# tomer196/GaUDI

Hardware: AMD Instinct MI355X
Metric: guided molecules/sec (1000-step) (higher is better)
Workload: dtype f32

## Files before the change

gaudi_amd/csrc/w8_nodes_f16.h:

```cpp
#pragma once
#include "w8_split.h"

namespace gaudi {
namespace w8 {


constexpr float kLoScale = 2048.f;
#ifndef GAUDI_NODE_ABLATE
#define GAUDI_NODE_ABLATE 0
#endif
constexpr int kAblateH = GAUDI_NODE_ABLATE;
#ifndef GAUDI_NODE_STAMPS
#define GAUDI_NODE_STAMPS 0
#endif
#ifndef GAUDI_NODE_PRIO
#define GAUDI_NODE_PRIO 1
#endif
struct NodeStampH {
  unsigned long long sum[8], last;
  __device__ __forceinline__ void start() { last = __builtin_amdgcn_s_memtime(); }
  __device__ __forceinline__ void mark(int i) {
    const unsigned long long t = __builtin_amdgcn_s_memtime();
    sum[i] += t - last;
    last = t;
// ... 140 lines not shown
  NodeSetH<NodeGeoH<HP>::NTW> s[NodeGeoH<HP>::D];
};

constexpr int kOOBBytes = (int)0x80000000u;
template <int HP>
struct TileLanesH {
  int vo[NodeGeoH<HP>::NTW];
  __device__ __forceinline__ TileLanesH(int wave, int lane, bool on = true) {
#pragma unroll
    for (int u = 0; u < NodeGeoH<HP>::NTW; ++u)
      vo[u] = (on && wave + kWaves * u < NodeGeoH<HP>::T) ? lane * 16 + (wave + kWaves * u) * 2048 : kOOBBytes;
  }
};
template <int HP, int NU = NodeGeoH<HP>::NTW>
__device__ __forceinline__ void nh_load(NodeSetH<NodeGeoH<HP>::NTW>& s, const WBuf& wh, int chunk_off, const TileLanesH<HP>& tl) {
#pragma unroll
  for (int u = 0; u < NU; ++u) {
    s.p[u][0] = __builtin_bit_cast(u4, __builtin_amdgcn_raw_buffer_load_b128(wh.r, tl.vo[u], chunk_off * 4, GAUDI_NODE_LOAD_AUX));
    s.p[u][1] = __builtin_bit_cast(u4, __builtin_amdgcn_raw_buffer_load_b128(wh.r, tl.vo[u] + 1024, chunk_off * 4, GAUDI_NODE_LOAD_AUX));
  }
}
constexpr int kAheadOne = 1, kAheadAll = 99;
template <int HP, int AHEAD = kAheadAll, int NU = 0>
__device__ __forceinline__ void node_prefetch_h(NodePFH<HP>& pf, const WBuf& wh, int W , int wave, int lane) {
  constexpr int nd = AHEAD < NodeGeoH<HP>::D ? AHEAD : NodeGeoH<HP>::D;
  const TileLanesH<HP> tl(wave, lane);
  static_for<nd>([&](auto d_tag) {
    constexpr int d = decltype(d_tag)::value;
    nh_load<HP, (NU > 0 ? NU : NodeGeoH<HP>::NTW)>(pf.s[d], wh, 2 * W + d * nh_chunk_floats(HP), tl);
  });
}

constexpr int kNodePlain = 0;
constexpr int kNodeFresh = 1;
constexpr int kNodeOneTile = 2;
constexpr int kNodeSlots1 = 4, kNodeSlots2 = 8;
__host__ __device__ constexpr bool node_one_tile(int FL) { return (FL & 3) == kNodeOneTile; }
template <int HP>
__host__ __device__ constexpr bool node_uneven_slots() { return NodeGeoH<HP>::NTW == 2 && NodeGeoH<HP>::T < 2 * kWaves; }
template <int HP>
__host__ __device__ constexpr int node_slots(int FL) { return node_one_tile(FL) && node_uneven_slots<HP>() ? FL >> 2 : 0; }
constexpr int kTailRuntime = 0;
constexpr int kTailOne = 1;

struct NodeCtxH {
  float winv;
  float* split_a;
  float* split_b;
  bool ktail;
  float* scales;
  float* scales_b = nullptr;
};

struct YInitBias {};
struct YInitRows {
  const float* y;
};
template <int HP, int EPI, bool TWO, int MAXNT, int PIN = kAheadOne, int POUT = kAheadOne, int FL = kNodePlain, int TAIL = kTailRuntime,
          int NU = 0, class XB = const float*, class XA = const float*, class YI = YInitBias>
__device__ __forceinline__ void node_gemm_h(const WBuf& wh, int Wa, const XA& sXa, bool do_split_a, int Wb, const XB& sXb,
                                            const float* sBias, float* sY, const float* sRes, const float* sMask, int N, int wave,
                                            int lane, const NodeCtxH& cx, NodePFH<HP>& pf, int nextW = -1, float* gPre = nullptr,
                                            uint32_t* sMaxOut = nullptr ,
                                            NodeStampH* ns = nullptr, const YI& yinit = YI{}) {
  (void)ns;
  (void)yinit;
  using G = NodeGeoH<HP>;
  constexpr int T = G::T, LD = HP + 4, NTW = NU > 0 ? NU : G::NTW, nc = G::nc, D = G::D;
  constexpr int kIn = PIN < D ? PIN : D, kOut = POUT < D ? POUT : D;
  constexpr int TQ = TAIL == kTailOne ? 1 : 4;
  const bool ktail = TAIL == kTailOne ? true : cx.ktail;
  constexpr bool kFresh = FL == kNodeFresh;
  const int c = lane & 15, g = lane >> 4;
  const int nt = (MAXNT < 2 || N <= 16) ? 1 : (MAXNT < 3 || N <= 32) ? 2 : 3;
  const bool seq = TWO && cx.split_b == cx.split_a;
  const SplitBufH sa{cx.split_a, nt, cx.scales}, sb{cx.split_b, nt, cx.scales_b != nullptr ? cx.scales_b : cx.scales + kScaleFloatsH};
  const int bpos = nh_bpos(c, g);
  const TileLanesH<HP> tl(wave, lane);
  const TileLanesH<HP> tl_next(wave, lane, nextW >= 0);
  const int Wn = nextW >= 0 ? nextW : Wa;
  static_for<D>([&](auto d_tag) {
    constexpr int d = decltype(d_tag)::value;
    if constexpr (d >= kIn) nh_load<HP, NTW>(pf.s[d], wh, 2 * Wa + d * nh_chunk_floats(HP), tl);
  });
  float ta[NTW][TQ], tb[NTW][TQ];
  if constexpr (G::odd) {
#pragma unroll
    for (int u = 0; u < NTW; ++u) {
      const int t = wave + kWaves * u < T ? wave + kWaves * u : 0;
#pragma unroll
      for (int q = 0; q < TQ; ++q) {
        const int ln = ((q == 0 || !ktail) && wave + kWaves * u < T) ? lane : kOOBLane;
        ta[u][q] = __builtin_bit_cast(float, __builtin_amdgcn_raw_buffer_load_b32(wh.r, ln * 4, (2 * Wa + nh_tail_off(HP) + t * 256 + q * 64) * 4, 0));
        if constexpr (TWO)
          tb[u][q] = __builtin_bit_cast(float, __builtin_amdgcn_raw_buffer_load_b32(wh.r, ln * 4, (2 * Wb + nh_tail_off(HP) + t * 256 + q * 64) * 4, 0));
      }
    }
  }
  NSTAMP(0);
  if (!(kAblateH & 1)) {
    const int ls = kFresh ? fresh(lane) : lane;
    if (do_split_a) split_rows_h<HP>(sa, rows_of(sXa), N, wave, ls);
    if (TWO && !seq) split_rows_h<HP>(sb, sXb, N, wave, ls);
    NSTAMP(1);
    if (do_split_a || (TWO && !seq)) lds_barrier();
    NSTAMP(2);
  }

  f4 acc0[MAXNT][NTW], acc1[MAXNT][NTW], y[MAXNT][NTW];
#pragma unroll
  for (int j = 0; j < MAXNT; ++j)
#pragma unroll
    for (int u = 0; u < NTW; ++u) {
      const int t = wave + kWaves * u < T ? wave + kWaves * u : 0;
      acc0[j][u] = splat(0.f);
      acc1[j][u] = splat(0.f);
      y[j][u] = sBias != nullptr ? *(const f4*)(sBias + 16 * t + 4 * g) : splat(0.f);
      if constexpr (std::is_same<YI, YInitRows>::value)
        y[j][u] = j * 16 + c < N ? *(const f4*)(yinit.y + (j * 16 + c) * LD + 16 * t + 4 * g) : splat(0.f);
// ... 3 lines not shown
  };
  auto bld = [&](const SplitBufH& s_, int i, int j) {
    const float* q = s_.chunk(i) + bpos + j * 512;
    return BH{*(const u4*)q, *(const u4*)(q + 256)};
  };
  auto mm = [&](const NodeSetH<G::NTW>& s, const BH& b, int j) {
    if (kAblateH & 2) {
      asm volatile("" ::"v"(s.p[0][0]), "v"(s.p[0][1]), "v"(s.p[NTW - 1][0]), "v"(s.p[NTW - 1][1]), "v"(b.h), "v"(b.l));
      return;
    }
#pragma unroll
    for (int u = 0; u < NTW; ++u) acc1[j][u] = mfma_h(s.p[u][0], b.l, acc1[j][u]);
#pragma unroll
    for (int u = 0; u < NTW; ++u) acc0[j][u] = mfma_h(s.p[u][0], b.h, acc0[j][u]);
#pragma unroll
    for (int u = 0; u < NTW; ++u) acc1[j][u] = mfma_h(s.p[u][1], b.h, acc1[j][u]);
  };
  auto tail_steps = [&](const SplitBufH& s_, const float (&tw)[NTW][TQ], auto j_tag) {
    constexpr int j = decltype(j_tag)::value;
    if constexpr (G::odd) {
      const float* xt = s_.tail(HP) + j * 256 + g * 16 + c;
#pragma unroll
      for (int u = 0; u < NTW; ++u) y[j][u] = mfma1(tw[u][0], xt[0], y[j][u]);
      if constexpr (TQ > 1) {
        if (!ktail) {
#pragma unroll
          for (int q = 1; q < TQ; ++q)
#pragma unroll
            for (int u = 0; u < NTW; ++u) y[j][u] = mfma1(tw[u][q], xt[64 * q], y[j][u]);
        }
      }
    }
  };
  auto fold = [&](const SplitBufH& s_, const float (&tw)[NTW][TQ]) {
    static_for<MAXNT>([&](auto j_tag) {
      constexpr int j = decltype(j_tag)::value;
      if (j < nt) {
        tail_steps(s_, tw, j_tag);
        const float sc = s_.scale(HP)[j * 16 + c] * cx.winv;
#pragma unroll
        for (int u = 0; u < NTW; ++u) {
          y[j][u] = y[j][u] + (acc0[j][u] + acc1[j][u] * (1.0f / kLoScale)) * sc;
          acc0[j][u] = splat(0.f);
          acc1[j][u] = splat(0.f);
        }
      }
    });
  };
  auto source = [&](auto src_tag, const SplitBufH& s_) {
    constexpr int src = decltype(src_tag)::value;
    constexpr bool last_src = !TWO || src == 1;
    const int Wcur = src == 0 ? Wa : Wb;
    BH bcur = bld(s_, 0, 0);
    static_for<nc>([&](auto i_tag) {
      constexpr int i = decltype(i_tag)::value;
      constexpr int d = i % D;
      BH bnext = bcur;
      if constexpr (i + 1 < nc) bnext = bld(s_, i + 1, 0);
      __builtin_amdgcn_sched_barrier(0);
      mm(pf.s[d], bcur, 0);
      if constexpr (MAXNT >= 2) {
        if (nt >= 2) {
          mm(pf.s[d], bld(s_, i, 1), 1);
          if constexpr (MAXNT >= 3) {
            if (nt >= 3) mm(pf.s[d], bld(s_, i, 2), 2);
          }
        }
      }
      __builtin_amdgcn_sched_barrier(0);
      if (!(kAblateH & 4)) {
        if constexpr (i + D < nc) nh_load<HP, NTW>(pf.s[d], wh, 2 * Wcur + (i + D) * nh_chunk_floats(HP), tl);
        else if constexpr (!last_src) nh_load<HP, NTW>(pf.s[d], wh, 2 * Wb + d * nh_chunk_floats(HP), tl);
        else if constexpr (d < kOut) nh_load<HP, NTW>(pf.s[d], wh, 2 * Wn + d * nh_chunk_floats(HP), tl_next);
      }
      __builtin_amdgcn_sched_barrier(0);
      bcur = bnext;
    });
  };
  NSTAMP(3);
#if GAUDI_NODE_PRIO
  if constexpr (!kFresh)
    if ((GAUDI_NODE_PRIO == 1 && wave >= kWaves / 2) || (GAUDI_NODE_PRIO == 2 && wave < kWaves / 2)) __builtin_amdgcn_s_setprio(1);
#endif
  source(std::integral_constant<int, 0>{}, sa);
  NSTAMP(4);
  fold(sa, ta);
  NSTAMP(5);
  if constexpr (TWO) {
    if (seq) {
      lds_barrier();
      split_rows_h<HP>(sb, sXb, N, wave, kFresh ? fresh(lane) : lane);
      lds_barrier();
    }
    source(std::integral_constant<int, 1>{}, sb);
    fold(sb, tb);
  }
#if GAUDI_NODE_PRIO
  if constexpr (!kFresh) __builtin_amdgcn_s_setprio(0);
#endif
  const int le = kFresh ? fresh(lane) : lane, ce = le & 15, ge = le >> 4;
  static_for<MAXNT>([&](auto j_tag) {
    constexpr int j = decltype(j_tag)::value;
    if (j < nt) {
#pragma unroll
      for (int u = 0; u < NTW; ++u) {
        const int t = wave + kWaves * u;
        const int nd = j * 16 + ce;
        f4 yy = y[j][u];
        if (t < T && nd < N) {
          float* dst = sY + nd * LD + 16 * t + 4 * ge;
          const bool pad = G::odd && ktail && t == T - 1 && ge > 0;
          if (pad) yy = splat(0.f);
          if (gPre != nullptr) nstash_store((f4*)(gPre + nd * HP + 16 * t + 4 * ge), yy);
          if (sMaxOut != nullptr) atomicMax(sMaxOut + nd, umax(umax(absbits(yy[0]), absbits(yy[1])), umax(absbits(yy[2]), absbits(yy[3]))));
          if (!pad) {
            if (EPI == EPI_SILU) yy = silu4v(yy);
            if (EPI == EPI_RESIDUAL_MASK) {
              const f4 r = *(const f4*)(sRes + nd * LD + 16 * t + 4 * ge);
              yy = (r + yy) * sMask[nd];
            }
            if (EPI == EPI_MUL_DSILU) {
              const f4 r = *(const f4*)(sRes + nd * LD + 16 * t + 4 * ge);
              yy = yy * dsilu4v(r);
            }
            if (EPI == EPI_ACCUM) yy = *(const f4*)(sRes + nd * LD + 16 * t + 4 * ge) + yy;
          }
          *(f4*)dst = yy;
        }
// ... 74 lines not shown
        f4 y = a.bias != nullptr ? *(const f4*)(a.bias + 16 * t + 4 * g) : splat(0.f);
        if constexpr (G::odd) y = mfma1(job.tw[u], xt, y);
        y = y + (job.acc0[u] + job.acc1[u] * (1.0f / kLoScale)) * sc;
        if (c < a.N) *(f4*)(a.out + c * LD + 16 * t + 4 * g) = y;
      });
    }
  }
}
template <int HP, int S>
__device__ __forceinline__ void side_rest(SideJobH<HP>& job, const SideArgsH& a, int lane) {
  if constexpr (S < SideGeoH<HP>::kSteps) {
    side_compute<HP, S>(job, a, lane);
    __builtin_amdgcn_sched_barrier(0);
    side_issue<HP, S + 1>(job, a, lane);
    side_rest<HP, S + 1>(job, a, lane);
  }
}
template <int HP, int MODE, int S0>
__device__ __forceinline__ void side_trips(RingS<HP, MODE>& ring, const WBuf& wb, int W, int nextW, int lane, SideJobH<HP>& job,
                                           const SideArgsH& a) {
  static_for<side_trip_count<HP, MODE>()>([&](auto tr_tag) {
    constexpr int tr = decltype(tr_tag)::value, s = S0 + tr;
    side_barrier<SideGeoH<HP>::loads(s)>();
    RingsStageSide<HP, MODE, tr>::run(ring, wb, W, nextW, lane);
    __builtin_amdgcn_sched_barrier(0);
    side_compute<HP, s>(job, a, lane);
    __builtin_amdgcn_sched_barrier(0);
    side_issue<HP, s + 1>(job, a, lane);
    __builtin_amdgcn_sched_barrier(0);
    ring.par ^= 1;
  });
}

#ifndef GAUDI_NODE_F16
#define GAUDI_NODE_F16 1
#endif
template <int SP>
struct NodeMath {
  static constexpr bool kF16 = SP != 0 && GAUDI_NODE_F16 != 0;
};
template <int HP, bool NH>
struct NodePFSel {
  using type = NodePF<HP>;
};
template <int HP>
struct NodePFSel<HP, true> {
  using type = NodePFH<HP>;
};
template <int HP, bool NH, int AHEAD, int FL = kNodePlain, class PF>
__device__ __forceinline__ void node_prefetch_x(PF& pf, const WBuf& wb, const WBuf& wbe, int W, int N, int wave, int lane, bool tw) {
  if constexpr (NH) node_prefetch_h<HP, AHEAD, node_slots<HP>(FL)>(pf, wbe, W, wave, lane);
  else node_prefetch<HP>(pf, wb, W, wave, lane, tw);
}
template <int HP, int EPI, bool TWO, int GN, bool NH, int PIN, int POUT, int FL = kNodePlain, int XBS = 0, class PF>
__device__ __forceinline__ void node_gemm_x(const WBuf& wb, const WBuf& wbe, int Wa, const float* Xa, const float* XaS, bool split_a, int Wb,
                                            const float* Xb, const float* XbS, const float* sBias, float* sY, const float* sRes,
                                            const float* sMask, int N, int wave, int lane, bool tw, const NodeCtxH& cx, PF& pf,
                                            int nextW = -1, float* gPre = nullptr, uint32_t* sMaxOut = nullptr,
                                            const float* Xb1 = nullptr, float xb_div = 1.f) {
  static_assert(XBS == 0 || (NH && GN == 0 && TWO), "summed second sources: the fp16-pair form of the resident kernels");
  if constexpr (NH) {
    constexpr int MAXNT = GN ? 3 : node_one_tile(FL) ? 1 : 2;
    constexpr int TAIL = node_one_tile(FL) && nh_odd(HP) ? kTailOne : kTailRuntime;
    constexpr int NU = node_slots<HP>(FL);
    if constexpr (XBS == 0)
      node_gemm_h<HP, EPI, TWO, MAXNT, PIN, POUT, FL, TAIL, NU>(wbe, Wa, Xa, split_a, Wb, Xb, sBias, sY, sRes, sMask, N, wave, lane, cx, pf, nextW,
                                                                gPre, sMaxOut);
    else
      node_gemm_h<HP, EPI, TWO, MAXNT, PIN, POUT, FL, TAIL, NU>(wbe, Wa, Xa, split_a, Wb, RowsSum<XBS == 2>{Xb, Xb1, xb_div}, sBias, sY, sRes, sMask,
                                                                N, wave, lane, cx, pf, nextW, gPre, sMaxOut);
  } else if constexpr (GN != 0) {
    node_gemm_n<HP, EPI, true, 3>(wb, Wa, XaS, Wb, XbS, sBias, sY, sRes, sMask, N, wave, lane, tw, &pf, nextW, gPre);
  } else {
    node_gemm<HP, EPI, true>(wb, Wa, Xa, Wb, Xb, sBias, sY, sRes, sMask, N, wave, lane, tw, &pf, nextW, gPre);
  }
}
__host__ __device__ constexpr bool node_ring_idle(int HP, int SP, bool GN) {
  return GN || (SP != 0 && GAUDI_NODE_F16 != 0 && (SP == 2 || HP < 48));
}
template <int HP>
__device__ __forceinline__ NodeCtxH node_ctx_h(float* region, int cap, int N, float winv, bool ktail, float* scales) {
  const int nct = N <= 16 ? 1 : N <= 32 ? 2 : 3;
  const int need = nh_split_floats(HP, nct);
  return NodeCtxH{winv, region, 2 * need <= cap ? region + need : region, ktail, scales};
}
__host__ __device__ constexpr int nh_keep_floats(int HP, int N) { return nh_split_floats(HP, N <= 16 ? 1 : N <= 32 ? 2 : 3) + kScaleFloatsH; }
template <int HP>
__device__ __forceinline__ NodeCtxH node_ctx_keep(const NodeCtxH& cx, float* keep, int N) {
  const int nct = N <= 16 ? 1 : N <= 32 ? 2 : 3;
  return NodeCtxH{cx.winv, keep + kScaleFloatsH, cx.split_a, cx.ktail, keep, cx.scales};
  (void)nct;
}

}
}
```

gaudi_amd/csrc/w8_pred.h:

```cpp
#pragma once
#include "pred_device.h"
#include "w8_edm.h"

namespace gaudi {
namespace w8 {

template <int HP, int SP = 0, int GN = 0, bool PG = false>
struct PredSmem {
  static_assert(!(PG && GN != 0), "PG is a variant of the resident kernels");
  static_assert(!GN || SP != 0, "global node buffers: split edge GEMMs only (the fp32 form's publish buffer starts in b0 / b1)");
  static constexpr bool kGlobalNodes = GN != 0;
  float *b2, *b3, *b4;
  float *b0, *b1;
  float* ring;
  float* pub;
  float *x, *x0, *dx;
  uint32_t *pmax, *qmax;
  float* hsc;
  f4* geo;
  float *d0, *trans, *dd0;
  float* pred;
  float* vec;
  float* hk = nullptr;
  float* side = nullptr;
  __host__ __device__ static int floats(int N, int S, int pubx) {
    return EdgeRing<HP, SP>::kFloats + (GN ? gn_lds_buffers(GN) : PG ? 4 : 5) * N * (HP + 4) + pubx + 12 * N + 2 * align4(N) + 96 + S * 10 + 32 + 10 * HP;
  }
  __device__ __forceinline__ float* publish() const { return GN ? ring : b0; }
  __device__ void carve(float* base, int N, int S, int pubx, float* gnode = nullptr) {
    constexpr int LD = HP + 4;
    if (SP == 0) { ring = base; base += EdgeRing<HP, SP>::kFloats; }
    if (GN || PG) gnode = assume_global(gnode);
    float*& nb = GN ? gnode : base;
    if (GN == 2) { b2 = base; base += N * LD; } else { b2 = nb; nb += N * LD; }
    b3 = nb; nb += N * LD;
    if (PG) { b4 = gnode; gnode += N * LD; } else { b4 = nb; nb += N * LD; }
    b0 = nb; nb += N * LD;
    if (GN == 2) { b1 = base; base += N * LD; } else { b1 = nb; nb += N * LD; }
    if (SP != 0) { ring = base; base += EdgeRing<HP, SP>::kFloats; }
    pub = base; base += pubx;
    x = base; base += 4 * N;
    x0 = base; base += 4 * N;
    dx = base; base += 4 * N;
    pmax = (uint32_t*)base; base += align4(N);
    qmax = (uint32_t*)base; base += align4(N);
    hsc = base; base += 96;
    geo = (f4*)base; base += S * 4;
    d0 = base; base += S;
    trans = base; base += S * 4;
    dd0 = base; base += S;
    pred = base; base += 32;
    vec = base;
  }
};

// ... 212 lines not shown
    STAMP(ST_BARRIER);
    vec_prefetch<NV, kThreads>(vpf, wb, PredLayerW::vec_off(lay.layer(l + 1 < W.L ? l + 1 : l), HP), PredLayerW::vec_count(HP), tid);
    if constexpr (STG) {
      stage_rows(xs0, p, N * LD, wave, lane);
      stage_wait();
    }
    node_gemm_x<HP, EPI_RESIDUAL_MASK, false, GN, NH, kAheadOne, kAheadOne, FL>(wb, wbe, Lw.Wn2, p, xs0, true, -1, nullptr, nullptr, Lw.bn2, h, h, mg.mask, mg.NC, wave,
                                                     lane, tw, hctx(), pf, l + 1 < W.L ? lay.layer(l + 1) : -1);
    if (!last) coord_update(sm, mg, 1.0f, tid);
    STAMP(ST_NODE);
    __syncthreads();
    STAMP(ST_BARRIER);
  }
  {
    const float* ow = w + lay.out_w();
    const float* ob = w + lay.out_b();
    const float* msk = mg.mask;
    small_dots<kThreads>(
        N * K, HP, tid, [=](int qq, int f) { return gload(ow + (qq % K) * HP + f); },
        [=](int qq, int f) { return h[(qq / K) * LD + f]; },
        [=](int qq, float acc) { p[qq] = (acc + gload(ob + qq % K)) * msk[qq / K]; });
    __syncthreads();
    if (tid < K) {
      float s = 0.f;
      for (int n = 0; n < N; ++n) s += p[n * K + tid];
      sm.pred[tid] = s / readout_div;
    }
    __syncthreads();
  }
  STAMP(ST_X0);
}

template <int HP, int SP = 0, bool MR = false, int GN = 0, int FL = 0, class SM = PredSmem<HP, SP, GN>>
__device__ __forceinline__ void pred_backward(const PredDev& W, const MolGraph& mg, const SM& sm, const float* stash,
                                              float* sGrad, float readout_div, int pub_ch, int tid STAMP_DECL, const float* sZin = nullptr) {
  constexpr int LD = HP + 4;
  constexpr int T = HP / 16;
  const int wave = __builtin_amdgcn_readfirstlane(tid >> 6), lane = tid & 63, c = lane & 15, g = lane >> 4;
  const int N = mg.N, D = mg.D, F = W.F, F1 = F + 1, K = W.K, S = mg.S;
  PredLayout lay{HP, F1, K, W.L};
  const float* __restrict__ w = W.w;
  const WBuf wb = make_wbuf(W.w, W.w_bytes);
  const WBuf wbe = SP ? make_wbuf(W.ws, W.ws_bytes) : wb;
  const bool tw = W.ktail != 0;
  float *B0 = sm.b0, *B1 = sm.b1, *B2 = sm.b2, *dh = sm.b3, *B4 = sm.b4;
  const int tid_ = tid;
  float* pub = sm.publish();
  const int PLD = 16 * pub_ch + 4;
  const float* estash = stash + pred_stash_node_floats(N, HP, W.L);
  const float* astash = estash + (size_t)W.L * S * HP * 2;
  const float* pstash = astash + (size_t)W.L * S;
  const float* dpred = sm.pred + 16;
  const int nslots = mg.ntiles * 16;
  f4* dus = (f4*)const_cast<float*>(pstash + (size_t)W.L * S);

  if (sZin != nullptr) {
    for (int idx = tid; idx < N * 3; idx += kThreads) {
      const int n = idx / 3, d = idx % 3;
      const float v = sZin[n * D + d] * mg.mask[n];
      sm.x[4 * n + d] = v;
      sm.x0[4 * n + d] = v;
    }
    __syncthreads();
    compute_geo(sm, mg, 0.f, tid, true);
    __syncthreads();
  }
  {
    const float* ow = w + lay.out_w();
    for (int idx = tid; idx < N * HP; idx += kThreads) {
      const int n = idx / HP, f = idx % HP;
      float acc = 0.f;
      for (int k = 0; k < K; ++k) acc += (dpred[k] / readout_div) * gload(ow + k * HP + f);
      dh[n * LD + f] = acc * mg.mask[n];
    }
    for (int idx = tid; idx < N * 4; idx += kThreads) sm.dx[idx] = 0.f;
    for (int idx = tid; idx < S; idx += kThreads) sm.dd0[idx] = 0.f;
  }
  __syncthreads();

  typename EdgeRing<HP, SP>::type ring;
  er_init<HP>(ring, sm.ring, W.ktail != 0, W.ws, W.hinv);
  constexpr bool NH = NodeMath<SP>::kF16;
  constexpr bool RI = node_ring_idle(HP, SP, GN);
  constexpr bool STG = GN && !NH;
  float* const xs0 = sm.ring;
  float* const xs1 = sm.ring + stage_stride(N * LD);
  if constexpr (!RI) {
    const int L0 = lay.layer(W.L - 1);
    er_start<HP>(ring, wbe, L0 + 9 * HP * HP , wave, lane);
  }
  typename NodePFSel<HP, NH>::type pf;
  node_prefetch_x<HP, NH, kAheadOne, FL>(pf, wb, wbe, lay.layer(W.L - 1) + 13 * HP * HP , mg.NC, wave, lane, tw);
  auto hctx = [&]() {
    if constexpr (NH) {
      if constexpr (RI) return node_ctx_h<HP>(sm.ring, EdgeRing<HP, SP>::kFloats, mg.NC, W.hinv, tw, sm.hsc);
      else return node_ctx_h<HP>(ring.slot(ring.par ^ 1), EdgeRing<HP, SP>::kFloats / 2, mg.NC, W.hinv, tw, sm.hsc);
    } else {
      return NodeCtxH{1.f, nullptr, nullptr, tw, nullptr};
    }
  };
  constexpr int NV = (PredLayerW::vec_count(HP) + kThreads - 1) / kThreads;
  VecPF<NV> vpf;
  vec_prefetch<NV, kThreads>(vpf, wb, PredLayerW::vec_off(lay.layer(W.L - 1), HP), PredLayerW::vec_count(HP), tid);
  STAMP(ST_X1);
  for (int l = W.L - 1; l >= 0; --l) {
    const bool last = l == W.L - 1;
    const PredLayerW Lw(w, lay.layer(l), HP, sm.vec);
    const float* st = stash + (size_t)l * (3 * N * HP + 4 * N);
    {
      const int tid = fresh(tid_);
      const int n4 = N * (HP / 4);
#ifdef GAUDI_DIAG_HOT_STASH
      const f4* sp = (const f4*)W.w;
      const f4* sq = (const f4*)(W.w + N * HP);
      const f4* sn = (const f4*)(W.w + 2 * N * HP);
#else
      const f4* sp = (const f4*)st;
      const f4* sq = (const f4*)(st + N * HP);
      const f4* sn = (const f4*)(st + 2 * N * HP);
#endif
      const int i0 = tid < n4 ? tid : n4 - 1, i1 = tid + kThreads < n4 ? tid + kThreads : n4 - 1;
      const f4 xv = gload4((const f4*)(st + 3 * N * HP) + (tid < N ? tid : N - 1));
      const f4 p0 = nstash_load(sp + i0), q0 = nstash_load(sq + i0), v0 = nstash_load(sn + i0);
      const f4 p1 = nstash_load(sp + i1), q1 = nstash_load(sq + i1), v1 = nstash_load(sn + i1);
      vec_commit<NV, kThreads>(vpf, sm.vec, PredLayerW::vec_count(HP), tid);
      STAMP(ST_GUIDE);
      auto put = [&](int idx, f4 pv, f4 qv, f4 nv) {
        const int n = idx / (HP / 4), f = 4 * (idx % (HP / 4));
        *(f4*)(B2 + n * LD + f) = pv;
        *(f4*)(B1 + n * LD + f) = qv;
        *(f4*)(B4 + n * LD + f) = nv;
        *(f4*)(dh + n * LD + f) = *(const f4*)(dh + n * LD + f) * mg.mask[n];
      };
      if (tid < N) {
        *(f4*)(sm.x + 4 * tid) = xv;
        *(f4*)(sm.dx + 4 * tid) = *(const f4*)(sm.dx + 4 * tid) * mg.mask[tid];
      }
      if (tid < n4) put(tid, p0, q0, v0);
      if (tid + kThreads < n4) put(tid + kThreads, p1, q1, v1);
      for (int idx = tid + 2 * kThreads; idx < n4; idx += kThreads) put(idx, nstash_load(sp + idx), nstash_load(sq + idx), nstash_load(sn + idx));
      for (int idx = tid + kThreads; idx < N; idx += kThreads) {
        *(f4*)(sm.x + 4 * idx) = gload4((const f4*)(st + 3 * N * HP) + idx);
        *(f4*)(sm.dx + 4 * idx) = *(const f4*)(sm.dx + 4 * idx) * mg.mask[idx];
      }
    }
    STAMP(ST_PRED_IO);
    __syncthreads();
    if constexpr (STG) stage_rows(xs0, dh, N * LD, wave, lane);
    compute_geo(sm, mg, 1.0f, tid, false);
    if constexpr (STG) stage_wait();
    STAMP(ST_BWD_EDGE);
    node_gemm_x<HP, EPI_MUL_DSILU, false, GN, NH, kAheadOne, kAheadOne, FL>(wb, wbe, Lw.Wn2t, dh, xs0, true, -1, nullptr, nullptr, nullptr, STG ? xs1 : B4, B4, nullptr,
                                                 mg.NC, wave, lane, tw, hctx(), pf, Lw.Wn1ht);
    __syncthreads();
    {
      const NodeCtxH cx = hctx();
      node_gemm_x<HP, EPI_ACCUM, false, GN, NH, kAheadOne, kAheadAll, FL>(wb, wbe, Lw.Wn1ht, B4, xs1, true, -1, nullptr, nullptr, nullptr, dh, dh, nullptr, mg.NC,
                                                     wave, lane, tw, cx, pf, Lw.Wn1at);
      node_gemm_x<HP, EPI_NONE, false, GN, NH, kAheadAll, 0, FL>(wb, wbe, Lw.Wn1at, B4, xs1, false, -1, nullptr, nullptr, nullptr, B0, nullptr, nullptr,
                                                    mg.NC, wave, lane, tw, cx, pf);
    }
    __syncthreads();
    STAMP(ST_BWD_NODE);
    if constexpr (RI) er_start<HP>(ring, wbe, last ? Lw.W2t : Lw.Wc1t, wave, lane);
    {
      constexpr bool mr = MR;
      int rd = 0;
    pred_bwd_round:
      const bool more = MR && rd + 1 < mg.rounds;
      const TileCols tc = load_tile(mg, MR ? rd : 0, wave, c);
      const int tile = tc.slot >> 4;
      const f4 gg = sm.geo[tc.slot];
      const float d0v = sm.d0[tc.slot];
      f4 du[T];
      float a = 0.f, tau = 0.f, dtx = 0.f, dty = 0.f, dtz = 0.f;
      {
        f4 de[T];
        if (tc.active) {
          a = gload(astash + (size_t)l * S + tc.slot);
          dtx = sm.dx[4 * tc.i + 0];
          dty = sm.dx[4 * tc.i + 1];
          dtz = sm.dx[4 * tc.i + 2];
        }
        if (!last) {
          f4 cp[T];
          if (tc.active) {
#ifdef GAUDI_DIAG_HOT_STASH
            const f4* sc = (const f4*)(W.w + (size_t)tile * (T * 256)) + lane;
#else
            const f4* sc = (const f4*)(estash + edge_stash_off8(l, tile, 1, S, HP)) + lane;
#endif
#pragma unroll
            for (int t = 0; t < T; ++t) cp[t] = stash_load(sc + t * 64);
            const float phi = gload(pstash + (size_t)l * S + tc.slot);
            const float th = tanhf(phi);
            tau = W.use_tanh ? th * W.coords_range_layer : phi;
            const float dtau = (dtx * gg[1] + dty * gg[2] + dtz * gg[3]) * tc.mk;
            const float dphi = W.use_tanh ? dtau * W.coords_range_layer * (1.0f - th * th) : dtau;
#pragma unroll
            for (int t = 0; t < T; ++t)
              cp[t] = *(const f4*)(Lw.wc2 + 16 * t + 4 * g) * dphi * cp[t];
          } else {
#pragma unroll
            for (int t = 0; t < T; ++t) cp[t] = splat(0.f);
          }
          STAMP(ST_B_DCP);
          er_gemm_regs<HP>(de, cp, ring, wbe, Lw.Wc1t, Lw.W2t, nullptr, B0 + tc.i * LD ,
                             tc.active, wave, lane);
          STAMP(ST_B_DE);
        } else {
#pragma unroll
          for (int t = 0; t < T; ++t) de[t] = *(const f4*)(B0 + tc.i * LD + 16 * t + 4 * g);
        }
        if (tc.active) {
          f4 ve[T];
#ifdef GAUDI_DIAG_HOT_STASH
          const f4* sv = (const f4*)(W.w + (size_t)(8 + tile) * (T * 256)) + lane;
#else
          const f4* sv = (const f4*)(estash + edge_stash_off8(l, tile, 0, S, HP)) + lane;
#endif
#pragma unroll
          for (int t = 0; t < T; ++t) ve[t] = stash_load(sv + t * 64);
          float dadot = 0.f;
#pragma unroll
          for (int t = 0; t < T; ++t) dadot += dot4(de[t], silu4v(ve[t]));
          const float da = reduce_groups(dadot) * tc.mk;
          const float ds = W.attention ? da * a * (1.0f - a) : 0.f;
          const float am = a * tc.mk;
#pragma unroll
          for (int t = 0; t < T; ++t)
            de[t] = (de[t] * am + *(const f4*)(Lw.wa + 16 * t + 4 * g) * ds) * dsilu4v(ve[t]);
        }
        STAMP(ST_B_DV);
        er_gemm_regs<HP>(du, de, ring, wbe, Lw.W2t,
                         more ? (last ? Lw.W2t : Lw.Wc1t) : ((SP == 0 && l > 0) ? lay.layer(l - 1) + 10 * HP * HP : -1), nullptr, nullptr,
                         tc.active, wave, lane);
        STAMP(ST_B_DT1);
      }
      if (tc.active) {
        const float* pp = B2 + tc.i * LD + 4 * g;
        const float* qq = B1 + tc.j * LD + 4 * g;
        float drdot = 0.f, dd0dot = 0.f;
#pragma unroll
        for (int t = 0; t < T; ++t) {
          const f4 u = edge_u(pp, qq, Lw.cr, Lw.cd, g, t, gg[0], d0v);
          du[t] = du[t] * dsilu4v(u);
          drdot += dot4(du[t], *(const f4*)(Lw.cr + 16 * t + 4 * g));
          dd0dot += dot4(du[t], *(const f4*)(Lw.cd + 16 * t + 4 * g));
        }
        const float dr = reduce_groups(drdot), dd0v = reduce_groups(dd0dot);
        if (g == 0) {
          const int i = tc.i, j = tc.j;
          const float fx = sm.x[4 * i + 0] - sm.x[4 * j + 0];
          const float fy = sm.x[4 * i + 1] - sm.x[4 * j + 1];
          const float fz = sm.x[4 * i + 2] - sm.x[4 * j + 2];
          const float nrm = sqrtf(gg[0] + 1e-8f), den = nrm + 1.0f;
          const float cx = dtx * tau * tc.mk, cy = dty * tau * tc.mk, cz = dtz * tau * tc.mk;
          const float k1 = (cx * fx + cy * fy + cz * fz) / (den * den * nrm);
          *(f4*)(sm.trans + 4 * tc.slot) = (f4){cx / den - fx * k1 + 2.0f * fx * dr, cy / den - fy * k1 + 2.0f * fy * dr,
                                                cz / den - fz * k1 + 2.0f * fz * dr, 0.f};
          sm.dd0[tc.slot] += dd0v;
        }
      }
      if constexpr (MR) {
        if (more) {
          if (tc.active) {
            f4* sd = dus + (size_t)tile * (T * 64) + lane;
#pragma unroll
            for (int t = 0; t < T; ++t) stash_store(sd + t * 64, du[t]);
          }
          ++rd;
          goto pred_bwd_round;
        }
      }
      STAMP(ST_B_DU);
// ... 192 lines not shown
```

gaudi_amd/csrc/w8_split.h:

```cpp
#pragma once
#include "w8_common.h"
#ifndef GAUDI_EDGE_PRIO
#define GAUDI_EDGE_PRIO 0
#endif


namespace gaudi {
namespace w8 {

typedef _Float16 h8 __attribute__((ext_vector_type(8)));
typedef _Float16 h2 __attribute__((ext_vector_type(2)));
typedef __attribute__((ext_vector_type(2))) float f2;
typedef __attribute__((ext_vector_type(4))) uint32_t u4;
typedef __attribute__((ext_vector_type(2))) uint32_t u2;
constexpr int kPieces = 2;

template <int N, class F>
__device__ __forceinline__ void static_for(F f) {
  if constexpr (N > 0) {
    static_for<N - 1>(f);
    f(std::integral_constant<int, N - 1>{});
  }
}

// ... 250 lines not shown
  auto gen = [&](int m) {
    const f4 lo = silu4v(edge_u(pp, qq, sCr, sCd, g, 2 * m, r, d0));
    const f4 hi = 2 * m + 1 < T ? silu4v(edge_u(pp, qq, sCr, sCd, g, 2 * m + 1 < T ? 2 * m + 1 : 0, r, d0)) : splat(0.f);
    return split8(lo, hi, se);
  };
  B3 bin = gen(0), nb = bin;
  static_assert(G::NH <= 3, "at most three trips per K chunk");
  const bool tail = G::kTailOK && ring.ktail;
#if GAUDI_EDGE_PRIO & 1
  if (wave >= kWaves / 2) __builtin_amdgcn_s_setprio(1);
#endif
  auto chunk = [&](int m, const B3& bin, B3& nb) {
    const int mn = m + 1 < G::NC ? m + 1 : m;
    auto trip = [&](auto h_tag) {
      constexpr int h = decltype(h_tag)::value;
      constexpr int NT = G::tiles_of(h);
      const int tr = m * G::NH + h;
      trip_open(ring, lane);
      rings_mfma<HP, MODE, NT>(acc + h * G::CH, ring.slot(ring.par) + lane * 4, bin, active, [&] {
        rings_stage(ring, wb, W, nextW, tr, wave, lane);
        if (h == G::NH - 1) nb = gen(mn);
      });
      trip_close(ring, lane);
    };
    trip(std::integral_constant<int, 0>{});
    if constexpr (G::NH > 1) trip(std::integral_constant<int, 1>{});
    if constexpr (G::NH > 2) trip(std::integral_constant<int, 2>{});
  };
  const int full = tail ? G::NC - 1 : G::NC;
  int m = 0;
#pragma unroll 1
  for (; m + 1 < full; m += 2) {
    chunk(m, bin, nb);
    chunk(m + 1, nb, bin);
  }
  if (m < full) chunk(m, bin, nb);
  if constexpr (G::kTailOK) {
    if (tail) {
      trip_open(ring, lane);
      const float bt = silu_f(edge_u_tail(pp, qq, sCr, sCd, g, T, r, d0)[0]) * se;
      rings_mfma_tail<HP, MODE>(acc, ring.slot(ring.par) + lane * 4, bt, active,
                          [&] { rings_stage(ring, wb, W, nextW, G::kTripsTail - 1, wave, lane); });
      trip_close(ring, lane);
    }
  }
#if GAUDI_EDGE_PRIO & 1
  __builtin_amdgcn_s_setprio(0);
#endif
  const float dsc = sc.inv * ring.winv;
#pragma unroll
  for (int t = 0; t < T; ++t) acc[t] = acc[t] * dsc + *(const f4*)(sB2 + 16 * t + 4 * g);
}

template <int HP, int MODE>
__device__ __forceinline__ void edge_gemm_regs_s(f4 (&out)[HP / 16], const f4 (&in)[HP / 16], RingS<HP, MODE>& ring, const WBuf& wb,
                                                 int W, int nextW, const float* sBias, const float* rowinit, bool active,
                                                 int wave, int lane) {
  using G = SplitGeo<HP, MODE>;
  constexpr int T = G::T;
  const int g = lane >> 4;
  uint32_t mx = 0;
#pragma unroll
  for (int t = 0; t < T; ++t) {
    out[t] = splat(0.f);
    mx = umax(mx, umax(umax(absbits(in[t][0]), absbits(in[t][1])), umax(absbits(in[t][2]), absbits(in[t][3]))));
  }
  const Pow2Scale sc = scale_for(column_max(mx));
  const float se = sc.s;
  static_assert(G::NH <= 3, "at most three trips per K chunk");
  const int c = lane & 15;
#if GAUDI_EDGE_PRIO & 2
  if (wave >= kWaves / 2) __builtin_amdgcn_s_setprio(1);
#endif
  auto chunk = [&](auto m_tag) {
    constexpr int m = decltype(m_tag)::value;
    const B3 bin = split8(in[2 * m], 2 * m + 1 < T ? in[2 * m + 1 < T ? 2 * m + 1 : 0] : splat(0.f), se);
    auto trip = [&](auto h_tag) {
      constexpr int h = decltype(h_tag)::value;
      constexpr int tr = m * G::NH + h;
      trip_open(ring, lane);
      rings_mfma<HP, MODE, G::tiles_of(h)>(out + h * G::CH, ring.slot(ring.par) + lane * 4, bin, active,
                                           [&] { rings_stage(ring, wb, W, nextW, tr, wave, lane); });
      trip_close(ring, lane);
    };
    trip(std::integral_constant<int, 0>{});
    if constexpr (G::NH > 1) trip(std::integral_constant<int, 1>{});
    if constexpr (G::NH > 2) trip(std::integral_constant<int, 2>{});
  };
  auto finish = [&] {
#if GAUDI_EDGE_PRIO & 2
    __builtin_amdgcn_s_setprio(0);
#endif
    const float dsc = sc.inv * ring.winv;
#pragma unroll
    for (int t = 0; t < T; ++t) {
      f4 b = sBias != nullptr ? *(const f4*)(sBias + 16 * t + 4 * g) : splat(0.f);
      if (rowinit != nullptr) b = b + *(const f4*)(rowinit + 16 * t + 4 * g);
      out[t] = out[t] * dsc + b;
    }
  };
  static_for<G::NC - 1>([&](auto m_tag) { chunk(m_tag); });
  if constexpr (G::kTailOK) {
    if (ring.ktail) {
      trip_open(ring, lane);
      rings_mfma_tail<HP, MODE>(out, ring.slot(ring.par) + lane * 4, tail_to_b(in[T - 1], c, g)[0] * se, active,
                          [&] { rings_stage(ring, wb, W, nextW, G::kTripsTail - 1, wave, lane); });
      trip_close(ring, lane);
      finish();
      return;
    }
  }
  chunk(std::integral_constant<int, G::NC - 1>{});
  finish();
}

template <int HP, int SP>
struct EdgeRing {
  using type = RingS<HP, SP>;
  static constexpr int kFloats = 2 * SplitGeo<HP, SP>::kSlotFloats;
};
template <int HP>
struct EdgeRing<HP, 0> {
  using type = Ring<HP>;
  static constexpr int kFloats = 2 * (HP / 16) * 256;
};
__host__ __device__ constexpr int edge_ring_floats(int HP, int mode) {
  const int T = HP / 16;
  const int CH = (mode == 2 || (T + 1) / 2 == 1) && T > 1 ? (T + 1) / 2 : T;
  return mode ? 2 * CH * kPieces * 256 : 2 * T * 256;
}
static_assert(edge_ring_floats(32, 1) == EdgeRing<32, 1>::kFloats && edge_ring_floats(208, 1) == EdgeRing<208, 1>::kFloats &&
                  edge_ring_floats(48, 2) == EdgeRing<48, 2>::kFloats && edge_ring_floats(208, 2) == EdgeRing<208, 2>::kFloats,
              "host LDS planning and SplitGeo disagree");
__device__ __forceinline__ int split_off(int W) { return W < 0 ? -1 : 2 * W; }

template <int HP>
__device__ __forceinline__ void er_init(Ring<HP>& r, float* base, bool ktail, const float*, float) {
  r.base = base;
  r.par = 0;
  r.ktail = ktail;
}
template <int HP, int MODE>
__device__ __forceinline__ void er_init(RingS<HP, MODE>& r, float* base, bool ktail, const float* ws, float winv) {
  r.base = base;
  r.par = 0;
  r.ktail = ktail;
  r.gbase = ws;
  r.winv = winv;
}
template <int HP>
__device__ __forceinline__ void er_start(Ring<HP>& r, const WBuf& wb, int W, int wave, int lane) {
  ring_start<HP>(r, wb, W, wave, lane);
}
template <int HP, int MODE>
__device__ __forceinline__ void er_start(RingS<HP, MODE>& r, const WBuf& wb, int W, int wave, int lane) {
  rings_start(r, wb, split_off(W), wave, lane);
}
template <int HP>
__device__ __forceinline__ void er_gemm_pq(f4 (&acc)[HP / 16], Ring<HP>& ring, const WBuf& wb, int W, int nextW, const float* sB2,
                                           const float* sCr, const float* sCd, const float* pp, const float* qq, float r, float d0,
                                           float, bool active, int wave, int lane STAMP_DECL) {
  edge_gemm_pq<HP>(acc, ring, wb, W, nextW, sB2, sCr, sCd, pp, qq, r, d0, active, wave, lane STAMP_ARGS);
}
template <int HP, int MODE>
__device__ __forceinline__ void er_gemm_pq(f4 (&acc)[HP / 16], RingS<HP, MODE>& ring, const WBuf& wb, int W, int nextW, const float* sB2,
                                           const float* sCr, const float* sCd, const float* pp, const float* qq, float r, float d0,
                                           float ubound, bool active, int wave, int lane STAMP_DECL) {
  edge_gemm_pq_s(acc, ring, wb, split_off(W), split_off(nextW), sB2, sCr, sCd, pp, qq, r, d0, ubound, active, wave, lane);
}
template <int HP>
__device__ __forceinline__ void er_gemm_regs(f4 (&out)[HP / 16], const f4 (&in)[HP / 16], Ring<HP>& ring, const WBuf& wb, int W,
                                             int nextW, const float* sBias, const float* rowinit, bool active, int wave, int lane) {
  edge_gemm_regs<HP>(out, in, ring, wb, W, nextW, sBias, rowinit, active, wave, lane);
}
template <int HP, int MODE>
__device__ __forceinline__ void er_gemm_regs(f4 (&out)[HP / 16], const f4 (&in)[HP / 16], RingS<HP, MODE>& ring, const WBuf& wb, int W,
                                             int nextW, const float* sBias, const float* rowinit, bool active, int wave, int lane) {
  edge_gemm_regs_s(out, in, ring, wb, split_off(W), split_off(nextW), sBias, rowinit, active, wave, lane);
}

}
}
```

Before: 229.6.

## Ride edge-stash loads behind node GEMM and edge GEMM weight loads

Adds hook/ride callbacks that issue global loads of the edge stash rows (cp/ve tiles and phi) inside the node GEMM after its last weight load, and inside the edge GEMM at a chosen trip. The aim is to hide stash-load latency behind MFMA work instead of stalling before the backward edge stage. In one path a __syncthreads is relaxed to an LDS barrier, and a side_barrier replaces a trip_open. This raises register pressure (extra f4 arrays) and risks occupancy loss or sync subtleties.

```diff
diff --git a/gaudi_amd/csrc/w8_nodes_f16.h b/gaudi_amd/csrc/w8_nodes_f16.h
--- a/gaudi_amd/csrc/w8_nodes_f16.h
+++ b/gaudi_amd/csrc/w8_nodes_f16.h
@@ -216,19 +216,38 @@
   float* scales_b = nullptr;
 };
 
+struct NoHookH {
+  static constexpr bool kOn = false;
+  __device__ __forceinline__ void operator()() const {}
+};
+template <class F>
+struct HookH {
+  static constexpr bool kOn = true;
+  F f;
+  __device__ __forceinline__ void operator()() const { f(); }
+};
+template <class F>
+__device__ __forceinline__ HookH<F> hook_h(F f) { return HookH<F>{f}; }
+__host__ __device__ constexpr int nh_last_load(int nc, int D, int kOut) {
+  int r = -1;
+  for (int i = 0; i < nc; ++i)
+    if (i + D < nc || i % D < kOut) r = i;
+  return r;
+}
 struct YInitBias {};
 struct YInitRows {
   const float* y;
 };
 template <int HP, int EPI, bool TWO, int MAXNT, int PIN = kAheadOne, int POUT = kAheadOne, int FL = kNodePlain, int TAIL = kTailRuntime,
-          int NU = 0, class XB = const float*, class XA = const float*, class YI = YInitBias>
+          int NU = 0, class XB = const float*, class XA = const float*, class YI = YInitBias, class HOOK = NoHookH>
 __device__ __forceinline__ void node_gemm_h(const WBuf& wh, int Wa, const XA& sXa, bool do_split_a, int Wb, const XB& sXb,
                                             const float* sBias, float* sY, const float* sRes, const float* sMask, int N, int wave,
                                             int lane, const NodeCtxH& cx, NodePFH<HP>& pf, int nextW = -1, float* gPre = nullptr,
                                             uint32_t* sMaxOut = nullptr ,
-                                            NodeStampH* ns = nullptr, const YI& yinit = YI{}) {
+                                            NodeStampH* ns = nullptr, const YI& yinit = YI{}, const HOOK& hook = HOOK{}) {
   (void)ns;
   (void)yinit;
+  (void)hook;
   using G = NodeGeoH<HP>;
   constexpr int T = G::T, LD = HP + 4, NTW = NU > 0 ? NU : G::NTW, nc = G::nc, D = G::D;
   constexpr int kIn = PIN < D ? PIN : D, kOut = POUT < D ? POUT : D;
@@ -338,6 +357,10 @@
     constexpr bool last_src = !TWO || src == 1;
     const int Wcur = src == 0 ? Wa : Wb;
     BH bcur = bld(s_, 0, 0);
+    if constexpr (HOOK::kOn && last_src && nh_last_load(nc, D, kOut) < 0) {
+      hook();
+      __builtin_amdgcn_sched_barrier(0);
+    }
     static_for<nc>([&](auto i_tag) {
       constexpr int i = decltype(i_tag)::value;
       constexpr int d = i % D;
@@ -360,6 +383,10 @@
         else if constexpr (d < kOut) nh_load<HP, NTW>(pf.s[d], wh, 2 * Wn + d * nh_chunk_floats(HP), tl_next);
       }
       __builtin_amdgcn_sched_barrier(0);
+      if constexpr (HOOK::kOn && last_src && i == nh_last_load(nc, D, kOut)) {
+        hook();
+        __builtin_amdgcn_sched_barrier(0);
+      }
       bcur = bnext;
     });
   };
@@ -540,20 +567,21 @@
   if constexpr (NH) node_prefetch_h<HP, AHEAD, node_slots<HP>(FL)>(pf, wbe, W, wave, lane);
   else node_prefetch<HP>(pf, wb, W, wave, lane, tw);
 }
-template <int HP, int EPI, bool TWO, int GN, bool NH, int PIN, int POUT, int FL = kNodePlain, int XBS = 0, class PF>
+template <int HP, int EPI, bool TWO, int GN, bool NH, int PIN, int POUT, int FL = kNodePlain, int XBS = 0, class PF, class HOOK = NoHookH>
 __device__ __forceinline__ void node_gemm_x(const WBuf& wb, const WBuf& wbe, int Wa, const float* Xa, const float* XaS, bool split_a, int Wb,
                                             const float* Xb, const float* XbS, const float* sBias, float* sY, const float* sRes,
                                             const float* sMask, int N, int wave, int lane, bool tw, const NodeCtxH& cx, PF& pf,
                                             int nextW = -1, float* gPre = nullptr, uint32_t* sMaxOut = nullptr,
-                                            const float* Xb1 = nullptr, float xb_div = 1.f) {
+                                            const float* Xb1 = nullptr, float xb_div = 1.f, const HOOK& hook = HOOK{}) {
   static_assert(XBS == 0 || (NH && GN == 0 && TWO), "summed second sources: the fp16-pair form of the resident kernels");
+  static_assert(!HOOK::kOn || (NH && XBS == 0), "a hook rides behind the fp16-pair form's last weight load");
   if constexpr (NH) {
     constexpr int MAXNT = GN ? 3 : node_one_tile(FL) ? 1 : 2;
     constexpr int TAIL = node_one_tile(FL) && nh_odd(HP) ? kTailOne : kTailRuntime;
     constexpr int NU = node_slots<HP>(FL);
     if constexpr (XBS == 0)
-      node_gemm_h<HP, EPI, TWO, MAXNT, PIN, POUT, FL, TAIL, NU>(wbe, Wa, Xa, split_a, Wb, Xb, sBias, sY, sRes, sMask, N, wave, lane, cx, pf, nextW,
-                                                                gPre, sMaxOut);
+      node_gemm_h<HP, EPI, TWO, MAXNT, PIN, POUT, FL, TAIL, NU, const float*, const float*, YInitBias, HOOK>(
+          wbe, Wa, Xa, split_a, Wb, Xb, sBias, sY, sRes, sMask, N, wave, lane, cx, pf, nextW, gPre, sMaxOut, nullptr, YInitBias{}, hook);
     else
       node_gemm_h<HP, EPI, TWO, MAXNT, PIN, POUT, FL, TAIL, NU>(wbe, Wa, Xa, split_a, Wb, RowsSum<XBS == 2>{Xb, Xb1, xb_div}, sBias, sY, sRes, sMask,
                                                                 N, wave, lane, cx, pf, nextW, gPre, sMaxOut);
diff --git a/gaudi_amd/csrc/w8_pred.h b/gaudi_amd/csrc/w8_pred.h
--- a/gaudi_amd/csrc/w8_pred.h
+++ b/gaudi_amd/csrc/w8_pred.h
@@ -1,6 +1,18 @@
 #pragma once
 #include "pred_device.h"
 #include "w8_edm.h"
+#ifndef GAUDI_STASH_RIDE
+#define GAUDI_STASH_RIDE 3
+#endif
+#ifndef GAUDI_RIDE_TILES
+#define GAUDI_RIDE_TILES 6
+#endif
+#ifndef GAUDI_HOOK_TILES
+#define GAUDI_HOOK_TILES 6
+#endif
+#ifndef GAUDI_STASH_RIDE_PLAIN
+#define GAUDI_STASH_RIDE_PLAIN 0
+#endif
 
 namespace gaudi {
 namespace w8 {
@@ -319,6 +331,12 @@
   const float* pstash = astash + (size_t)W.L * S;
   const float* dpred = sm.pred + 16;
   const int nslots = mg.ntiles * 16;
+  constexpr bool kRide = SP == 1 && !MR && GN == 0 && SplitGeo<HP, SP == 1 ? 1 : 2>::kTailOK &&
+                         (node_one_tile(FL) || (GAUDI_STASH_RIDE_PLAIN && FL != kNodeFresh));
+  constexpr bool kRideA = kRide && (GAUDI_STASH_RIDE & 1), kRideB = kRide && (GAUDI_STASH_RIDE & 2);
+  constexpr int kHookTiles = GAUDI_HOOK_TILES < T ? GAUDI_HOOK_TILES : T;
+  constexpr int kRideTiles = GAUDI_RIDE_TILES < T ? GAUDI_RIDE_TILES : T;
+  constexpr int kRideTrip = SplitGeo<HP, SP == 1 ? 1 : 2>::kTripsTail - 2;
   f4* dus = (f4*)const_cast<float*>(pstash + (size_t)W.L * S);
 
   if (sZin != nullptr) {
@@ -420,14 +438,36 @@
     node_gemm_x<HP, EPI_MUL_DSILU, false, GN, NH, kAheadOne, kAheadOne, FL>(wb, wbe, Lw.Wn2t, dh, xs0, true, -1, nullptr, nullptr, nullptr, STG ? xs1 : B4, B4, nullptr,
                                                  mg.NC, wave, lane, tw, hctx(), pf, Lw.Wn1ht);
     __syncthreads();
+    f4 er[kHookTiles];
+    float rphi = 0.f;
+    auto edge_rows = [=](int tile, int which) {
+#ifdef GAUDI_DIAG_HOT_STASH
+      return (const f4*)(W.w + (size_t)((which ? 0 : 8) + tile) * (T * 256)) + lane;
+#else
+      return (const f4*)(estash + edge_stash_off8(l, tile, which, S, HP)) + lane;
+#endif
+    };
     {
       const NodeCtxH cx = hctx();
       node_gemm_x<HP, EPI_ACCUM, false, GN, NH, kAheadOne, kAheadAll, FL>(wb, wbe, Lw.Wn1ht, B4, xs1, true, -1, nullptr, nullptr, nullptr, dh, dh, nullptr, mg.NC,
                                                      wave, lane, tw, cx, pf, Lw.Wn1at);
-      node_gemm_x<HP, EPI_NONE, false, GN, NH, kAheadAll, 0, FL>(wb, wbe, Lw.Wn1at, B4, xs1, false, -1, nullptr, nullptr, nullptr, B0, nullptr, nullptr,
-                                                    mg.NC, wave, lane, tw, cx, pf);
-    }
-    __syncthreads();
+      if constexpr (kRideB) {
+        node_gemm_x<HP, EPI_NONE, false, GN, NH, kAheadAll, 0, FL>(
+            wb, wbe, Lw.Wn1at, B4, xs1, false, -1, nullptr, nullptr, nullptr, B0, nullptr, nullptr, mg.NC, wave, lane, tw, cx, pf, -1,
+            nullptr, nullptr, nullptr, 1.f, hook_h([&] {
+              const int rtile = wave < mg.ntiles ? wave : 0;
+              const f4* sr = edge_rows(rtile, last ? 0 : 1);
+              rphi = gload(pstash + (size_t)l * S + rtile * 16 + c);
+#pragma unroll
+              for (int t = 0; t < kHookTiles; ++t) er[t] = stash_load(sr + t * 64);
+            }));
+      } else {
+        node_gemm_x<HP, EPI_NONE, false, GN, NH, kAheadAll, 0, FL>(wb, wbe, Lw.Wn1at, B4, xs1, false, -1, nullptr, nullptr, nullptr, B0, nullptr, nullptr,
+                                                      mg.NC, wave, lane, tw, cx, pf);
+      }
+    }
+    if constexpr (kRideB) lds_barrier();
+    else __syncthreads();
     STAMP(ST_BWD_NODE);
     if constexpr (RI) er_start<HP>(ring, wbe, last ? Lw.W2t : Lw.Wc1t, wave, lane);
     {
@@ -442,7 +482,7 @@
       f4 du[T];
       float a = 0.f, tau = 0.f, dtx = 0.f, dty = 0.f, dtz = 0.f;
       {
-        f4 de[T];
+        f4 de[T], ve[T];
         if (tc.active) {
           a = gload(astash + (size_t)l * S + tc.slot);
           dtx = sm.dx[4 * tc.i + 0];
@@ -452,14 +492,11 @@
         if (!last) {
           f4 cp[T];
           if (tc.active) {
-#ifdef GAUDI_DIAG_HOT_STASH
-            const f4* sc = (const f4*)(W.w + (size_t)tile * (T * 256)) + lane;
-#else
-            const f4* sc = (const f4*)(estash + edge_stash_off8(l, tile, 1, S, HP)) + lane;
-#endif
-#pragma unroll
-            for (int t = 0; t < T; ++t) cp[t] = stash_load(sc + t * 64);
-            const float phi = gload(pstash + (size_t)l * S + tc.slot);
+            const f4* sc = edge_rows(tile, 1);
+#pragma unroll
+            for (int t = 0; t < T; ++t) cp[t] = (kRideB && t < kHookTiles) ? er[t] : stash_load(sc + t * 64);
+            if constexpr (kRideB) __builtin_amdgcn_sched_barrier(0);
+            const float phi = kRideB ? rphi : gload(pstash + (size_t)l * S + tc.slot);
             const float th = tanhf(phi);
             tau = W.use_tanh ? th * W.coords_range_layer : phi;
             const float dtau = (dtx * gg[1] + dty * gg[2] + dtz * gg[3]) * tc.mk;
@@ -472,22 +509,37 @@
             for (int t = 0; t < T; ++t) cp[t] = splat(0.f);
           }
           STAMP(ST_B_DCP);
-          er_gemm_regs<HP>(de, cp, ring, wbe, Lw.Wc1t, Lw.W2t, nullptr, B0 + tc.i * LD ,
+          if constexpr (kRideA) {
+            er_gemm_regs<HP>(de, cp, ring, wbe, Lw.Wc1t, Lw.W2t, nullptr, B0 + tc.i * LD, tc.active, wave, lane,
+                             ride_at<kRideTiles, kRideTrip>([&] {
+                               const f4* sv = edge_rows(tile, 0);
+#pragma unroll
+                               for (int t = 0; t < kRideTiles; ++t) ve[t] = stash_load(sv + t * 64);
+                             }));
+          } else {
+            er_gemm_regs<HP>(de, cp, ring, wbe, Lw.Wc1t, Lw.W2t, nullptr, B0 + tc.i * LD ,
                              tc.active, wave, lane);
+          }
           STAMP(ST_B_DE);
         } else {
 #pragma unroll
           for (int t = 0; t < T; ++t) de[t] = *(const f4*)(B0 + tc.i * LD + 16 * t + 4 * g);
         }
         if (tc.active) {
-          f4 ve[T];
-#ifdef GAUDI_DIAG_HOT_STASH
-          const f4* sv = (const f4*)(W.w + (size_t)(8 + tile) * (T * 256)) + lane;
-#else
-          const f4* sv = (const f4*)(estash + edge_stash_off8(l, tile, 0, S, HP)) + lane;
-#endif
-#pragma unroll
-          for (int t = 0; t < T; ++t) ve[t] = stash_load(sv + t * 64);
+          if constexpr (kRideA || kRideB) {
+            const f4* sv = edge_rows(tile, 0);
+            if (last) {
+#pragma unroll
+              for (int t = 0; t < T; ++t) ve[t] = (kRideB && t < kHookTiles) ? er[t] : stash_load(sv + t * 64);
+            } else {
+#pragma unroll
+              for (int t = kRideA ? kRideTiles : 0; t < T; ++t) ve[t] = stash_load(sv + t * 64);
+            }
+          } else {
+            const f4* sv = edge_rows(tile, 0);
+#pragma unroll
+            for (int t = 0; t < T; ++t) ve[t] = stash_load(sv + t * 64);
+          }
           float dadot = 0.f;
 #pragma unroll
           for (int t = 0; t < T; ++t) dadot += dot4(de[t], silu4v(ve[t]));
diff --git a/gaudi_amd/csrc/w8_split.h b/gaudi_amd/csrc/w8_split.h
--- a/gaudi_amd/csrc/w8_split.h
+++ b/gaudi_amd/csrc/w8_split.h
@@ -326,10 +326,23 @@
   for (int t = 0; t < T; ++t) acc[t] = acc[t] * dsc + *(const f4*)(sB2 + 16 * t + 4 * g);
 }
 
-template <int HP, int MODE>
+struct NoRide {
+  static constexpr int K = 0, R = -1;
+  __device__ __forceinline__ void operator()() const {}
+};
+template <int K_, int R_, class F>
+struct RideAt {
+  static constexpr int K = K_, R = R_;
+  F f;
+  __device__ __forceinline__ void operator()() const { f(); }
+};
+template <int K, int R, class F>
+__device__ __forceinline__ RideAt<K, R, F> ride_at(F f) { return RideAt<K, R, F>{f}; }
+
+template <int HP, int MODE, class RIDE = NoRide>
 __device__ __forceinline__ void edge_gemm_regs_s(f4 (&out)[HP / 16], const f4 (&in)[HP / 16], RingS<HP, MODE>& ring, const WBuf& wb,
                                                  int W, int nextW, const float* sBias, const float* rowinit, bool active,
-                                                 int wave, int lane) {
+                                                 int wave, int lane, const RIDE& ride = RIDE{}) {
   using G = SplitGeo<HP, MODE>;
   constexpr int T = G::T;
   const int g = lane >> 4;
@@ -346,15 +359,38 @@
 #if GAUDI_EDGE_PRIO & 2
   if (wave >= kWaves / 2) __builtin_amdgcn_s_setprio(1);
 #endif
+  static_assert(RIDE::K == 0 || (RIDE::R >= 0 && RIDE::R + 1 <= (G::NC - 1) * G::NH), "a ride sits in a full chunk's trip, with a trip after it");
+  auto open = [&](auto tr_tag) {
+    constexpr int tr = decltype(tr_tag)::value;
+    if constexpr (RIDE::K > 0 && tr == RIDE::R + 1) {
+      if (active) side_barrier<RIDE::K>();
+      else trip_barrier();
+    } else {
+      trip_open(ring, lane);
+    }
+  };
   auto chunk = [&](auto m_tag) {
     constexpr int m = decltype(m_tag)::value;
     const B3 bin = split8(in[2 * m], 2 * m + 1 < T ? in[2 * m + 1 < T ? 2 * m + 1 : 0] : splat(0.f), se);
     auto trip = [&](auto h_tag) {
       constexpr int h = decltype(h_tag)::value;
       constexpr int tr = m * G::NH + h;
-      trip_open(ring, lane);
-      rings_mfma<HP, MODE, G::tiles_of(h)>(out + h * G::CH, ring.slot(ring.par) + lane * 4, bin, active,
-                                           [&] { rings_stage(ring, wb, W, nextW, tr, wave, lane); });
+      open(std::integral_constant<int, tr>{});
+      if constexpr (RIDE::K > 0 && tr == RIDE::R) {
+        if (active)
+          rings_mfma_act<HP, MODE, G::tiles_of(h), true>(out + h * G::CH, ring.slot(ring.par) + lane * 4, bin, [&] {
+            rings_stage(ring, wb, W, nextW, tr, wave, lane);
+            __builtin_amdgcn_sched_barrier(0);
+            ride();
+            __builtin_amdgcn_sched_barrier(0);
+          });
+        else
+          rings_mfma_act<HP, MODE, G::tiles_of(h), false>(out + h * G::CH, ring.slot(ring.par) + lane * 4, bin,
+                                                          [&] { rings_stage(ring, wb, W, nextW, tr, wave, lane); });
+      } else {
+        rings_mfma<HP, MODE, G::tiles_of(h)>(out + h * G::CH, ring.slot(ring.par) + lane * 4, bin, active,
+                                             [&] { rings_stage(ring, wb, W, nextW, tr, wave, lane); });
+      }
       trip_close(ring, lane);
     };
     trip(std::integral_constant<int, 0>{});
@@ -376,7 +412,7 @@
   static_for<G::NC - 1>([&](auto m_tag) { chunk(m_tag); });
   if constexpr (G::kTailOK) {
     if (ring.ktail) {
-      trip_open(ring, lane);
+      open(std::integral_constant<int, G::kTripsTail - 1>{});
       rings_mfma_tail<HP, MODE>(out, ring.slot(ring.par) + lane * 4, tail_to_b(in[T - 1], c, g)[0] * se, active,
                           [&] { rings_stage(ring, wb, W, nextW, G::kTripsTail - 1, wave, lane); });
       trip_close(ring, lane);
@@ -447,11 +483,12 @@
                                              int nextW, const float* sBias, const float* rowinit, bool active, int wave, int lane) {
   edge_gemm_regs<HP>(out, in, ring, wb, W, nextW, sBias, rowinit, active, wave, lane);
 }
-template <int HP, int MODE>
+template <int HP, int MODE, class RIDE = NoRide>
 __device__ __forceinline__ void er_gemm_regs(f4 (&out)[HP / 16], const f4 (&in)[HP / 16], RingS<HP, MODE>& ring, const WBuf& wb, int W,
-                                             int nextW, const float* sBias, const float* rowinit, bool active, int wave, int lane) {
-  edge_gemm_regs_s(out, in, ring, wb, split_off(W), split_off(nextW), sBias, rowinit, active, wave, lane);
-}
-
-}
-}
+                                             int nextW, const float* sBias, const float* rowinit, bool active, int wave, int lane,
+                                             const RIDE& ride = RIDE{}) {
+  edge_gemm_regs_s<HP, MODE, RIDE>(out, in, ring, wb, split_off(W), split_off(nextW), sBias, rowinit, active, wave, lane, ride);
+}
+
+}
+}
```

Result: faster. 233.7, median of 6 (+1.8%).
